# evfro/polara

Measured on AMD Instinct MI355X. Metric: users scored/sec + SVD build time, ML-20M rank-50 PureSVD, higher is better.
Workload: dtype bf16x3; 1 GPU; ML-20M-shaped synthetic 138493 x 26744, ~2e7 nnz, 10 levels (BASELINE.json metric / configs[2]), PureSVD rank=50, top-10, all users scored; n_items=26744, nnz=19975287, rank=50, topk=10, prune=True, launch=python, passes on 2 streams

## Files before the change

polara_amd/csrc/score.hip:

```cpp
#include "pk_common.h"
#include "pk_settle.h"
#include <math.h>
#include <stdlib.h>

typedef float f32x16 __attribute__((ext_vector_type(16)));
typedef __bf16 bf16x8 __attribute__((ext_vector_type(8)));

#define RING 16

#define PK_IDX_FLOOR (-2)
#define PK_TILE_NONE 0xffffffff00000000ull

template <int K, int J, int S>
constexpr unsigned long long pk_wave_stage_mask() {
    unsigned long long m = 0;
    for (int l = 0; l < 64; ++l) {
        const int i = l + 64 * S;
        if (((i & J) == 0) == ((i & K) == 0)) m |= 1ull << l;
    }
    return m;
}
template <int SLOTS, int K, int J>
__device__ __forceinline__ void pk_sort32_stage(unsigned (&key)[SLOTS]) {
    if constexpr (J >= 64) {
        const unsigned hi = key[0] > key[1] ? key[0] : key[1], lo = key[0] > key[1] ? key[1] : key[0];
        key[0] = hi;
        key[1] = lo;
    } else {
        unsigned other[SLOTS];
#pragma unroll
        for (int s = 0; s < SLOTS; ++s) other[s] = (unsigned)pk_lane_xor<J>((int)key[s]);
        {
            const unsigned hi = key[0] > other[0] ? key[0] : other[0], lo = key[0] > other[0] ? other[0] : key[0];
            key[0] = __builtin_amdgcn_inverse_ballot_w64(pk_wave_stage_mask<K, J, 0>()) ? hi : lo;
        }
        if constexpr (SLOTS == 2) {
            const unsigned hi = key[1] > other[1] ? key[1] : other[1], lo = key[1] > other[1] ? other[1] : key[1];
            key[1] = __builtin_amdgcn_inverse_ballot_w64(pk_wave_stage_mask<K, J, 1>()) ? hi : lo;
        }
    }
}
template <int SLOTS, int K, int J>
__device__ __forceinline__ void pk_sort32_merge(unsigned (&key)[SLOTS]) {
    pk_sort32_stage<SLOTS, K, J>(key);
    if constexpr (J > 1) pk_sort32_merge<SLOTS, K, (J >> 1)>(key);
}
template <int SLOTS, int K>
__device__ __forceinline__ void pk_sort32_levels(unsigned (&key)[SLOTS]) {
    if constexpr (K > 2) pk_sort32_levels<SLOTS, (K >> 1)>(key);
    pk_sort32_merge<SLOTS, K, (K >> 1)>(key);
}
template <int SLOTS>
__device__ __forceinline__ void pk_sort32_wave_desc(unsigned (&key)[SLOTS]) {
    static_assert(SLOTS == 1 || SLOTS == 2, "pk_sort32_wave_desc: 64 or 128 elements");
    pk_sort32_levels<SLOTS, 64 * SLOTS>(key);
}

template <int K, int J>
constexpr unsigned long long pk_half_stage_mask() {
    unsigned long long m = 0;
    for (int l = 0; l < 64; ++l) {
        const int t = l & 31;
        if (((t & J) == 0) == ((t & K) == 0)) m |= 1ull << l;
    }
    return m;
}
template <int K, int J>
__device__ __forceinline__ void pk_sort32_half_merge(unsigned &key) {
    const unsigned other = (unsigned)pk_lane_xor<J>((int)key);
    const unsigned hi = key > other ? key : other, lo = key > other ? other : key;
    key = __builtin_amdgcn_inverse_ballot_w64(pk_half_stage_mask<K, J>()) ? hi : lo;
    if constexpr (J > 1) pk_sort32_half_merge<K, (J >> 1)>(key);
}
template <int K>
__device__ __forceinline__ void pk_sort32_half_levels(unsigned &key) {
    if constexpr (K > 2) pk_sort32_half_levels<(K >> 1)>(key);
    pk_sort32_half_merge<K, (K >> 1)>(key);
}
__device__ __forceinline__ unsigned pk_float_order(float x) {
    const unsigned u = __float_as_uint(x);
    return (u & 0x80000000u) ? ~u : (u | 0x80000000u);
}

__device__ __forceinline__ unsigned pk_bf16_rne(float x) {
    unsigned u = __float_as_uint(x);
    u += 0x7fffu + ((u >> 16) & 1u);
    return u >> 16;
}
__device__ __forceinline__ void pk_split_bf16(float x, unsigned &hi, unsigned &lo) {
    hi = pk_bf16_rne(x);
    lo = pk_bf16_rne(x - __uint_as_float(hi << 16));
}

struct LaneState {
    int64_t sp;
    float tau;
    int cnt;
};
#define PK_LANE_DONE (-1)

__host__ __device__ constexpr bool pk_top_in_lds(int nstep, int kc) { return kc <= 32 || nstep > 8; }
__host__ __device__ constexpr int pk_ring_rows(int nstep, int kc) { return kc == 16 ? 8 : ((nstep > 8 && kc == 64) ? 2 * RING : RING); }
__host__ __device__ constexpr size_t pk_score_lds_bytes(int nstep, int kc) {
    return (size_t)(4 * pk_ring_rows(nstep, kc) * 64 + (pk_top_in_lds(nstep, kc) ? 4 * 32 * kc : 1)) * sizeof(uint2);
}
struct SeenDense {
    const unsigned *mask;
    const int32_t *skip;
    int tiles;
};

struct UserRows {
    const double *E;
    int64_t ld;
    int K;
    const double *extra;
    int64_t extra_ld;
    double extra_scale;
    float *bound_out;
};

struct SettleExit {
    int topk;
    double vmax;
    const float *item_norm;
    int64_t *out_idx;
    const int64_t *out_perm;
    int32_t *flags;
    int32_t *open_list;
    int32_t *open_count;
};

struct ExitCtx {
    SettleExit sx;
    const int64_t *seen_ptr;
    const double *extra;
    int64_t extra_ld;
    int64_t n_users;
    int K;
};
#define PK_EXIT_CTX_BYTES 128
static_assert(sizeof(ExitCtx) <= PK_EXIT_CTX_BYTES, "ExitCtx: one 128-byte LDS slot per wave");
__host__ __device__ constexpr size_t pk_score_settle_lds_bytes(int nstep, int kc) { return pk_score_lds_bytes(nstep, kc) + 4 * PK_EXIT_CTX_BYTES; }

template <int NSTEP, int KC, bool STRIDED, bool DENSE, bool SETTLE = false>
__global__ __launch_bounds__(256) void score_candidates_kernel(
    const float4 *__restrict__ Vp, const float4 *__restrict__ Ep, int64_t n_users, int n_items,
    int n_tiles, int split_tiles, int chunk_begin, int chunk_tiles,
    const int64_t *__restrict__ seen_ptr, const unsigned long long *__restrict__ seen_tiles,
    const int32_t *__restrict__ seen_ntiles,
    float *__restrict__ cand_score, int32_t *__restrict__ cand_idx,
    LaneState *__restrict__ st_lane, uint2 *__restrict__ st_ring,
    const float *__restrict__ user_bound, const float *__restrict__ tile_bound, SeenDense dense,
    int tile_base, int slot_base, const LaneState *__restrict__ floor_state, int boot_tiles, UserRows rows, SettleExit sx) {
    constexpr int KQ = 2 * NSTEP;
    constexpr bool PAIRED = (KC == 16);
    constexpr int RG = pk_ring_rows(NSTEP, KC);
    constexpr int SLOTS = (2 * RG + KC + 63) / 64;
    constexpr bool TOP_LDS = pk_top_in_lds(NSTEP, KC);
    extern __shared__ __attribute__((aligned(16))) uint2 pk_score_lds[];
    constexpr int NW = 4;

    const int lane = threadIdx.x & 63;
    const int wave = __builtin_amdgcn_readfirstlane((int)(threadIdx.x >> 6));
    const int64_t group_raw = (int64_t)blockIdx.x * NW + wave;
    if (group_raw * 32 >= n_users) return;
    const int64_t group = group_raw;
    uint2(*ring)[64] = reinterpret_cast<uint2(*)[64]>(pk_score_lds + wave * (RG * 64));
    uint2 *top = pk_score_lds + NW * RG * 64 + (TOP_LDS ? wave * (32 * KC) : 0);
    constexpr int CTX_AT = NW * RG * 64 + NW * 32 * KC;
    if constexpr (SETTLE) {
        if (lane == 0) {
            ExitCtx *cx = reinterpret_cast<ExitCtx *>(pk_score_lds + CTX_AT + wave * (PK_EXIT_CTX_BYTES / 8));
            cx->sx = sx;
            cx->seen_ptr = seen_ptr;
            cx->extra = rows.extra;
            cx->extra_ld = rows.extra_ld;
            cx->n_users = n_users;
            cx->K = rows.K;
        }
    }

    const int split = STRIDED ? (int)blockIdx.y : 0;
    const int S = STRIDED ? (int)gridDim.y : 1;
    const int64_t n_groups = (n_users + 31) / 32;
    const int t_lo = tile_base + split;
    const int tile_begin = t_lo + chunk_begin * S;
    const int tile_stop = (chunk_begin + chunk_tiles < split_tiles) ? t_lo + (chunk_begin + chunk_tiles) * S : n_tiles;
    const int tile_end = (tile_stop < n_tiles) ? tile_stop : n_tiles;
    const bool first = (chunk_begin == 0);
    const bool last = (tile_stop >= n_tiles);
    if (!first && tile_begin >= n_tiles) return;

    const int ul = lane & 31, hi = lane >> 5;
    const int64_t user = group * 32 + ul;
    const int64_t slot = (int64_t)(slot_base + split) * n_groups + group;
    float *my_score = cand_score + slot * 32 * KC;
    int32_t *my_idx = cand_idx + slot * 32 * KC;

    float4 e[KQ];
    float en_rows = -1.0f;
    if (rows.E) {
        double *buf = reinterpret_cast<double *>(&ring[0][0]);
        double ss = 0.0;
#pragma unroll
        for (int s = 0; s < NSTEP; ++s) {
            __builtin_amdgcn_wave_barrier();
#pragma unroll
            for (int p = 0; p < 4; ++p) {
                const int rr = 8 * p + (lane >> 3);
                const int kk = 16 * s + 2 * (lane & 7);
                const int64_t grow = group * 32 + rr;
                double2 v = make_double2(0.0, 0.0);
                if (grow < n_users && kk < rows.K) {
                    const double *g = rows.E + grow * rows.ld + kk;
                    if (kk + 1 < rows.K) v = *reinterpret_cast<const double2 *>(g);
                    else v.x = g[0];
                }
                *reinterpret_cast<double2 *>(buf + rr * 16 + 2 * (lane & 7)) = v;
            }
            __builtin_amdgcn_wave_barrier();
            unsigned bh[8], bl[8];
            const double *mine = buf + ul * 16 + 8 * hi;
#pragma unroll
            for (int j = 0; j < 8; ++j) {
                const double x = mine[j];
                ss = fma(x, x, ss);
                pk_split_bf16((float)x, bh[j], bl[j]);
            }
            e[2 * s] = __builtin_bit_cast(float4, make_uint4(bh[0] | (bh[1] << 16), bh[2] | (bh[3] << 16), bh[4] | (bh[5] << 16), bh[6] | (bh[7] << 16)));
            e[2 * s + 1] = __builtin_bit_cast(float4, make_uint4(bl[0] | (bl[1] << 16), bl[2] | (bl[3] << 16), bl[4] | (bl[5] << 16), bl[6] | (bl[7] << 16)));
        }
        __builtin_amdgcn_wave_barrier();
        ss += pk_lane_xor<32>(ss);
        if (user < n_users) {
            double b = sqrt(ss) * (1.0 + 1e-6);
            if (rows.extra) b += rows.extra_scale * rows.extra[user * rows.extra_ld];
            en_rows = (float)(b * (1.0 + 1e-7));
            if (rows.bound_out && chunk_begin == 0 && hi == 0 && (!STRIDED || blockIdx.y == 0)) rows.bound_out[user] = en_rows;
        }
    } else {
#pragma unroll
        for (int q = 0; q < KQ; ++q) e[q] = Ep[(group * KQ + q) * 64 + lane];
    }

    int64_t sp = 0, se = 0;
    unsigned long long nxt = PK_TILE_NONE, nxt2 = PK_TILE_NONE, nxt3 = PK_TILE_NONE;
    float tau = -INFINITY;
    int cnt = 0;
    const bool prune = (user_bound != nullptr || rows.E != nullptr) && tile_bound != nullptr;
    const float en = (prune && user < n_users) ? (rows.E ? en_rows : user_bound[user]) : -1.0f;
    bool pruned = false;
    int exit_tile = tile_end;
    const bool has_seen = (seen_ptr != nullptr && user < n_users);
    if (has_seen) {
        sp = seen_ptr[user];
        se = sp + seen_ntiles[user];
    }
    LaneState *my_state = st_lane + slot * 64 + lane;
    uint2 *my_ring_state = st_ring + slot * (RING * 64);
    float tau_floor = -INFINITY;
    if constexpr (STRIDED) {
        if (floor_state) {
            const LaneState fs = floor_state[group * 64 + lane];
            if ((int)fs.sp < tile_base) {
                if (first) {
                    for (int s = lane; s < 32 * KC; s += 64) {
                        my_score[s] = -INFINITY;
                        my_idx[s] = -1;
                    }
                    LaneState ls;
                    ls.sp = fs.sp;
                    ls.tau = fs.tau;
                    ls.cnt = PK_LANE_DONE;
                    *my_state = ls;
                }
                return;
            }
            tau_floor = fs.tau;
            tau = tau_floor;
        }
    }
    const int dense_tiles = (DENSE && seen_ptr != nullptr) ? dense.tiles : 0;
    const unsigned *dense_row = dense_tiles ? dense.mask + ((int64_t)group * dense_tiles) * 32 + ul : nullptr;
    if (DENSE && first && has_seen && dense_tiles) sp += dense.skip[user];
    if (first) {
        if (has_seen && t_lo > 0 && !(DENSE && dense_tiles >= t_lo)) {
            int64_t lo = sp, hi_ = se;
            while (lo < hi_) {
                const int64_t mid = (lo + hi_) >> 1;
                if ((unsigned)(seen_tiles[mid] >> 32) < (unsigned)t_lo) lo = mid + 1; else hi_ = mid;
            }
            sp = lo;
        }
        for (int s = lane; s < 32 * KC; s += 64) {
            if (TOP_LDS) {
                top[s] = make_uint2(__float_as_uint(-INFINITY), 0xffffffffu);
            } else {
                my_score[s] = -INFINITY;
                my_idx[s] = -1;
            }
        }
    } else {
        const LaneState ls = *my_state;
        if (ls.cnt == PK_LANE_DONE) {
            return;
        }
        if (TOP_LDS)
            for (int s = lane; s < 32 * KC; s += 64) top[s] = make_uint2(__float_as_uint(my_score[s]), (unsigned)my_idx[s]);
        if (has_seen) sp = ls.sp;
        tau = ls.tau;
        tau_floor = fmaxf(tau_floor, tau);
        cnt = ls.cnt;
        const int cmax = __builtin_amdgcn_readfirstlane((int)__reduce_max_sync(~0ull, cnt));
        for (int i = 0; i < cmax; ++i) ring[i][lane] = my_ring_state[i * 64 + lane];
    }
    if (has_seen) {
        if (sp < se) nxt = seen_tiles[sp];
        if (sp + 1 < se) nxt2 = seen_tiles[sp + 1];
        if (sp + 2 < se) nxt3 = seen_tiles[sp + 2];
    }

    auto flush_user = [&](int x) {
        if (TOP_LDS) {
            __builtin_amdgcn_wave_barrier();
        } else {
            __builtin_amdgcn_fence(__ATOMIC_RELEASE, "workgroup");
            __builtin_amdgcn_wave_barrier();
        }
        const int c_lo = __builtin_amdgcn_readlane(cnt, x);
        const int c_hi = __builtin_amdgcn_readlane(cnt, x + 32);
        if (!TOP_LDS) __builtin_amdgcn_fence(__ATOMIC_ACQUIRE, "workgroup");
        if constexpr (SLOTS == 2 && KC == 64) {
            constexpr unsigned SRC_MASK = 127u;
            float ka = -INFINITY, kb = -INFINITY;
            int va = PK_IDX_NONE, vb = PK_IDX_NONE;
            if (TOP_LDS) {
                const uint2 r = top[x * KC + lane];
                if ((int)r.y >= 0) {
                    ka = __uint_as_float(r.x);
                    va = (int)r.y;
                }
            } else {
                const int iv = my_idx[x * KC + lane];
                if (iv >= 0) {
                    ka = my_score[x * KC + lane];
                    va = iv;
                }
            }
            if (lane < RG) {
                if (lane < c_lo) {
                    const uint2 r = ring[lane][x];
                    kb = __uint_as_float(r.x);
                    vb = (int)r.y;
                }
            } else if (lane < 2 * RG) {
                if (lane - RG < c_hi) {
                    const uint2 r = ring[lane - RG][x + 32];
                    kb = __uint_as_float(r.x);
                    vb = (int)r.y;
                }
            }
            unsigned qa = (pk_float_order(ka) & ~SRC_MASK) | (unsigned)(127 - lane);
            unsigned qb[1] = {(pk_float_order(kb) & ~SRC_MASK) | (unsigned)lane};
            pk_sort32_wave_desc<1>(qb);
            const unsigned qr = (unsigned)__shfl((int)qb[0], 63 - lane, 64);
            unsigned q[1] = {qa > qr ? qa : qr};
            pk_sort32_merge<1, 64, 32>(q);
            const int code = (int)(q[0] & SRC_MASK);
            const int src = (code >= 64) ? 127 - code : code;
            const float fa = __shfl(ka, src, 64), fb = __shfl(kb, src, 64);
            const int ia = __shfl(va, src, 64), ib = __shfl(vb, src, 64);
            const float fk = (code >= 64) ? fa : fb;
            const int fv = (code >= 64) ? ia : ib;
            const int iv = (fv == PK_IDX_NONE) ? -1 : fv;
            if (TOP_LDS) {
                top[x * KC + lane] = make_uint2(__float_as_uint(fk), (unsigned)iv);
            } else {
                my_score[x * KC + lane] = fk;
                my_idx[x * KC + lane] = iv;
            }
            const float ntau = __int_as_float(__builtin_amdgcn_readlane(__float_as_int(fk), KC - 1));
            if (ul == x) {
                tau = fmaxf(ntau, tau_floor);
                cnt = 0;
            }
            __builtin_amdgcn_wave_barrier();
            return;
        }
        float key[SLOTS];
        int val[SLOTS];
#pragma unroll
        for (int s = 0; s < SLOTS; ++s) {
            const int i = lane + 64 * s;
            float k = -INFINITY;
            int v = PK_IDX_NONE;
            if (i < RG) {
                if (i < c_lo) {
                    uint2 r = ring[i][x];
                    k = __uint_as_float(r.x);
                    v = (int)r.y;
                }
            } else if (i < 2 * RG) {
                if (i - RG < c_hi) {
                    uint2 r = ring[i - RG][x + 32];
                    k = __uint_as_float(r.x);
                    v = (int)r.y;
                }
            } else if (i < 2 * RG + KC) {
                const int t = i - 2 * RG;
                if (TOP_LDS) {
                    const uint2 r = top[x * KC + t];
                    if ((int)r.y >= 0) {
                        k = __uint_as_float(r.x);
                        v = (int)r.y;
                    }
                } else {
                    const int iv = my_idx[x * KC + t];
                    if (iv >= 0) {
                        k = my_score[x * KC + t];
                        v = iv;
                    }
                }
            }
            key[s] = k;
            val[s] = v;
        }
        constexpr unsigned SRC_MASK = 64u * SLOTS - 1u;
        unsigned k32[SLOTS];
#pragma unroll
        for (int s = 0; s < SLOTS; ++s) k32[s] = (pk_float_order(key[s]) & ~SRC_MASK) | (unsigned)(lane + 64 * s);
        pk_sort32_wave_desc<SLOTS>(k32);
        {
            float ok[SLOTS];
            int ov[SLOTS];
#pragma unroll
            for (int s = 0; s < SLOTS; ++s) {
                const int src = (int)(k32[s] & SRC_MASK);
                float fk = __shfl(key[0], src & 63, 64);
                int fv = __shfl(val[0], src & 63, 64);
                if constexpr (SLOTS == 2) {
                    const float fk1 = __shfl(key[1], src & 63, 64);
                    const int fv1 = __shfl(val[1], src & 63, 64);
                    if (src >= 64) {
                        fk = fk1;
                        fv = fv1;
                    }
                }
                ok[s] = fk;
                ov[s] = fv;
            }
#pragma unroll
            for (int s = 0; s < SLOTS; ++s) {
                key[s] = ok[s];
                val[s] = ov[s];
            }
        }
#pragma unroll
        for (int s = 0; s < SLOTS; ++s) {
            const int i = lane + 64 * s;
            if (i < KC) {
                const int iv = (val[s] == PK_IDX_NONE) ? -1 : val[s];
                if (TOP_LDS) {
                    top[x * KC + i] = make_uint2(__float_as_uint(key[s]), (unsigned)iv);
                } else {
                    my_score[x * KC + i] = key[s];
                    my_idx[x * KC + i] = iv;
                }
            }
        }
        const float ntau = __int_as_float(
            __builtin_amdgcn_readlane(__float_as_int(key[(KC - 1) / 64]), (KC - 1) & 63));
        if (ul == x) {
            tau = fmaxf(ntau, tau_floor);
            cnt = 0;
        }
        __builtin_amdgcn_wave_barrier();
    };
    auto flush_pair = [&](int x, int y) {
        __builtin_amdgcn_wave_barrier();
        const int t = lane & 31;
        const int yy = (y >= 0) ? y : x;
        const int cx_lo = __builtin_amdgcn_readlane(cnt, x), cx_hi = __builtin_amdgcn_readlane(cnt, x + 32);
        const int cy_lo = __builtin_amdgcn_readlane(cnt, yy), cy_hi = __builtin_amdgcn_readlane(cnt, yy + 32);
        const int u = hi ? yy : x;
        const int c_lo = hi ? cy_lo : cx_lo, c_hi = hi ? cy_hi : cx_hi;
        const bool act = !hi || y >= 0;
        float k = -INFINITY;
        int v = PK_IDX_NONE;
        if (act) {
            if (t < KC) {
                const uint2 r = top[u * KC + t];
                if ((int)r.y >= 0) {
                    k = __uint_as_float(r.x);
                    v = (int)r.y;
                }
            } else if (t < KC + RG) {
                if (t - KC < c_lo) {
                    const uint2 r = ring[t - KC][u];
                    k = __uint_as_float(r.x);
                    v = (int)r.y;
                }
            } else if (t - KC - RG < c_hi) {
                const uint2 r = ring[t - KC - RG][u + 32];
                k = __uint_as_float(r.x);
                v = (int)r.y;
            }
        }
        unsigned key = (pk_float_order(k) & ~31u) | (unsigned)t;
        pk_sort32_half_levels<32>(key);
        const int src = (lane & 32) | (int)(key & 31u);
        k = __shfl(k, src, 64);
        v = __shfl(v, src, 64);
        if (act && t < KC) top[u * KC + t] = make_uint2(__float_as_uint(k), (unsigned)((v == PK_IDX_NONE) ? -1 : v));
        const float tx = __int_as_float(__builtin_amdgcn_readlane(__float_as_int(k), KC - 1));
        const float ty = __int_as_float(__builtin_amdgcn_readlane(__float_as_int(k), 32 + KC - 1));
        if (ul == x) {
            tau = fmaxf(tx, tau_floor);
            cnt = 0;
        }
        if (y >= 0 && ul == y) {
            tau = fmaxf(ty, tau_floor);
            cnt = 0;
        }
        __builtin_amdgcn_wave_barrier();
    };
    auto flush_set = [&](unsigned um) {
        if constexpr (PAIRED) {
            while (um) {
                const int x = __builtin_ctz(um);
                um &= um - 1;
                int y = -1;
                if (um) {
                    y = __builtin_ctz(um);
                    um &= um - 1;
                }
                flush_pair(x, y);
            }
        } else {
            while (um) {
                const int x = __builtin_ctz(um);
                um &= um - 1;
                flush_user(x);
            }
        }
    };

    auto load_frags = [&](int tile, float4(&dst)[KQ]) {
        const float4 *vp = Vp + ((int64_t)tile * KQ) * 64 + lane;
#pragma unroll
        for (int q = 0; q < KQ; ++q) dst[q] = vp[q * 64];
    };
    unsigned m_dense = 0;
    unsigned long long pend = PK_TILE_NONE;
    bool has_pend = false;
    auto take_pending = [&]() {
        if (has_pend) nxt3 = (sp + 2 < se) ? pend : PK_TILE_NONE;
        has_pend = false;
    };
    auto walk_mask = [&](int tile) -> unsigned {
        const int j0 = tile * 32, jend = j0 + 32;
        unsigned mask = 0;
        if constexpr (DENSE) {
            if (tile < dense_tiles) {
                mask = m_dense;
                if (jend > n_items) mask |= ~0u << (n_items - j0);
                return mask;
            }
        }
        if (S > 1) {
            while (__any((unsigned)(nxt >> 32) < (unsigned)tile)) {
                take_pending();
                if ((unsigned)(nxt >> 32) < (unsigned)tile) {
                    ++sp;
                    nxt = nxt2;
                    nxt2 = nxt3;
                    nxt3 = (sp + 2 < se) ? seen_tiles[sp + 2] : PK_TILE_NONE;
                }
            }
        }
        const bool hit = (unsigned)(nxt >> 32) == (unsigned)tile;
        if (__any(hit)) {
            take_pending();
            if (hit) {
                mask = (unsigned)nxt;
                ++sp;
                nxt = nxt2;
                nxt2 = nxt3;
                nxt3 = PK_TILE_NONE;
            }
            pend = seen_tiles[(hit && sp + 2 < se) ? sp + 2 : 0];
            has_pend = hit;
        }
        if (jend > n_items) mask |= ~0u << (n_items - j0);
        return mask;
    };
    auto push_candidates = [&](const float(&acc)[16], int j0) {
#pragma unroll
        for (int r = 0; r < 16; ++r) {
            bool c = acc[r] > tau;
            if (__any(c)) {
                if (__any(c && cnt == RG)) {
                    const unsigned long long full = __ballot(cnt == RG);
                    unsigned um = (unsigned)(full | (full >> 32));
                    if (PAIRED && (__builtin_popcount(um) & 1)) {
                        const unsigned long long part = __ballot(2 * cnt >= RG);
                        const unsigned cand = (unsigned)(part | (part >> 32)) & ~um;
                        if (cand) um |= 1u << __builtin_ctz(cand);
                    }
                    flush_set(um);
                    c = acc[r] > tau;
                }
                if (c) {
                    ring[cnt][lane] = make_uint2(__float_as_uint(acc[r]),
                                                 (unsigned)(j0 + (r & 3) + 8 * (r >> 2) + 4 * hi));
                    ++cnt;
                }
            }
        }
    };
    auto score_tile_roll = [&](float4(&a)[KQ], int next_tile) -> f32x16 {
        f32x16 acc;
#pragma unroll
        for (int r = 0; r < 16; ++r) acc[r] = 0.0f;
        const float4 *vp = Vp + ((int64_t)next_tile * KQ) * 64 + lane;
#pragma unroll
        for (int sidx = 0; sidx < NSTEP; ++sidx) {
            const bf16x8 vh = __builtin_bit_cast(bf16x8, a[2 * sidx]), vl = __builtin_bit_cast(bf16x8, a[2 * sidx + 1]);
            const bf16x8 eh = __builtin_bit_cast(bf16x8, e[2 * sidx]), el = __builtin_bit_cast(bf16x8, e[2 * sidx + 1]);
            acc = __builtin_amdgcn_mfma_f32_32x32x16_bf16(vh, eh, acc, 0, 0, 0);
            acc = __builtin_amdgcn_mfma_f32_32x32x16_bf16(vh, el, acc, 0, 0, 0);
            acc = __builtin_amdgcn_mfma_f32_32x32x16_bf16(vl, eh, acc, 0, 0, 0);
            a[2 * sidx] = vp[(2 * sidx) * 64];
            a[2 * sidx + 1] = vp[(2 * sidx + 1) * 64];
        }
        return acc;
    };
    if (first && boot_tiles > 0 && floor_state == nullptr) {
        constexpr int BL = KC / 2;
        constexpr int BG = KC / 8;
        float bl[BL];
#pragma unroll
        for (int i = 0; i < BL; ++i) bl[i] = -INFINITY;
        const int64_t sp0 = sp;
        const unsigned long long n0 = nxt, n1 = nxt2, n2 = nxt3;
        float4 a_nxt[KQ];
        load_frags((tile_begin < n_tiles) ? tile_begin : 0, a_nxt);
        unsigned m_nxt = 0u;
        if constexpr (DENSE) m_nxt = (tile_begin < dense_tiles) ? dense_row[(int64_t)tile_begin * 32] : 0u;
        for (int i = 0, tile = tile_begin; i < boot_tiles && tile < tile_end; ++i, tile += S) {
            {
                if constexpr (DENSE) {
                    m_dense = m_nxt;
                    m_nxt = (tile + S < dense_tiles) ? dense_row[(int64_t)(tile + S) * 32] : 0u;
                }
                f32x16 acc;
                acc = score_tile_roll(a_nxt, (tile + S < tile_end) ? tile + S : tile);
                const unsigned m2 = walk_mask(tile) >> (4 * hi);
#pragma unroll
                for (int g = 0; g < BG; ++g) {
                    float x = -INFINITY;
#pragma unroll
                    for (int r = g * (16 / BG); r < (g + 1) * (16 / BG); ++r)
                        x = fmaxf(x, (m2 & (1u << ((r & 3) + 8 * (r >> 2)))) ? -INFINITY : acc[r]);
#pragma unroll
                    for (int i2 = 0; i2 < BL; ++i2) {
                        const float up = fmaxf(bl[i2], x);
                        x = fminf(bl[i2], x);
                        bl[i2] = up;
                    }
                }
            }
        }
        float t0 = bl[KC / 2 - 1];
        t0 = fminf(t0, __int_as_float(pk_lane_xor<32>(__float_as_int(t0))));
        if (t0 > -INFINITY) {
            t0 = fminf(t0 - fabsf(t0) * 2.4e-7f, t0 - 1e-37f);
            tau_floor = fmaxf(tau_floor, t0);
            tau = fmaxf(tau, tau_floor);
        }
        sp = sp0;
        nxt = n0;
        nxt2 = n1;
        nxt3 = n2;
        has_pend = false;
    }
    {
        {
        float4 a_nxt[KQ];
        load_frags((tile_begin < n_tiles) ? tile_begin : 0, a_nxt);
        unsigned m_nxt = 0u;
        if constexpr (DENSE) m_nxt = (tile_begin < dense_tiles) ? dense_row[(int64_t)tile_begin * 32] : 0u;
        float tb = prune ? tile_bound[(tile_begin < n_tiles) ? tile_begin : 0] : 0.0f;
        int step = 0;
        for (int tile = tile_begin; tile < tile_end; tile += S, ++step) {
            if (prune) {
                const bool open = en * tb > tau;
                const unsigned long long ob = __ballot(open);
                if (ob == 0ull) {
                    pruned = true;
                    exit_tile = tile;
                    break;
                } else {
                    if (((STRIDED ? step : tile) & 7) == 7 && __popcll(ob) <= 16) {
                        const unsigned long long pend = __ballot(cnt > 0);
                        flush_set((unsigned)(ob | (ob >> 32)) & (unsigned)(pend | (pend >> 32)));
                    }
                    tb = tile_bound[(tile + S < n_tiles) ? tile + S : tile];
                }
            }
            {
                if constexpr (DENSE) {
                    m_dense = m_nxt;
                    m_nxt = (tile + S < dense_tiles) ? dense_row[(int64_t)(tile + S) * 32] : 0u;
                }
                f32x16 acc;
                acc = score_tile_roll(a_nxt, (tile + S < tile_end) ? tile + S : tile);
                const unsigned mask = walk_mask(tile);
                float m_all = fmaxf(acc[0], acc[1]);
#pragma unroll
                for (int r = 2; r < 16; ++r) m_all = fmaxf(m_all, acc[r]);
                if (__any(m_all > tau)) {
                    float sc[16];
                    float m = m_all;
                    if (__any(mask != 0)) {
                        const unsigned m2 = mask >> (4 * hi);
#pragma unroll
                        for (int r = 0; r < 16; ++r)
                            sc[r] = (m2 & (1u << ((r & 3) + 8 * (r >> 2)))) ? -INFINITY : acc[r];
                        m = fmaxf(sc[0], sc[1]);
#pragma unroll
                        for (int r = 2; r < 16; ++r) m = fmaxf(m, sc[r]);
                    } else {
#pragma unroll
                        for (int r = 0; r < 16; ++r) sc[r] = acc[r];
                    }
                    if (__any(m > tau)) push_candidates(sc, tile * 32);
                }
            }
        }
        }
    }

    if (!last && !pruned) {
        if constexpr (RG > RING) {
            const unsigned long long over = __ballot(cnt > RING);
            flush_set((unsigned)(over | (over >> 32)));
        }
        LaneState ls;
        ls.sp = sp;
        ls.tau = tau;
        ls.cnt = cnt;
        *my_state = ls;
        const int cmax = __builtin_amdgcn_readfirstlane((int)__reduce_max_sync(~0ull, cnt));
        __builtin_amdgcn_wave_barrier();
        for (int i = 0; i < cmax; ++i) my_ring_state[i * 64 + lane] = ring[i][lane];
        if (TOP_LDS)
            for (int s = lane; s < 32 * KC; s += 64) {
                const uint2 r = top[s];
                my_score[s] = __uint_as_float(r.x);
                my_idx[s] = (int)r.y;
            }
        return;
    }
    {
        const unsigned long long some = __ballot(cnt > 0);
        flush_set((unsigned)(some | (some >> 32)));
    }
    const unsigned long long floored = (floor_state == nullptr) ? __ballot(tau_floor > -INFINITY) : 0ull;
    unsigned settled_users = 0u;
    if constexpr (SETTLE) {
        static_assert(TOP_LDS && !STRIDED && (KC == 16 || KC == 32), "settle at exit: single sweep, lists in LDS, KC <= 32");
        constexpr int UPP = 64 / KC;
        const int sl = (int)__builtin_amdgcn_mbcnt_hi(~0u, __builtin_amdgcn_mbcnt_lo(~0u, 0u));
        int cx_at = CTX_AT + __builtin_amdgcn_readfirstlane((int)(threadIdx.x >> 6)) * (PK_EXIT_CTX_BYTES / 8);
        asm volatile("" : "+s"(cx_at));
        __builtin_amdgcn_wave_barrier();
        const ExitCtx cx = *reinterpret_cast<const ExitCtx *>(pk_score_lds + cx_at);
        const SettleExit &sx = cx.sx;
        const int64_t n_users = cx.n_users;
        const int64_t sgroup = (int64_t)blockIdx.x * NW + __builtin_amdgcn_readfirstlane((int)(threadIdx.x >> 6));
        const int su = sl & 31;
        const int64_t suser = sgroup * 32 + su;
        const int t = sl % KC, seg = sl / KC;
        double c_own = 0.0;
        int can_own = 0;
        int64_t irow_own = 0;
        if (suser < n_users) {
            c_own = pk_settle_coeff(cx.K, en, cx.extra[suser * cx.extra_ld]);
            const int64_t n_seen = cx.seen_ptr ? cx.seen_ptr[suser + 1] - cx.seen_ptr[suser] : 0;
            can_own = (n_items - n_seen >= sx.topk) ? 1 : 0;
            irow_own = sx.out_perm ? sx.out_perm[suser] : suser;
        }
        static_assert((size_t)RG * 64 * sizeof(uint2) >= (size_t)32 * KC * sizeof(float), "norms fit the ring area");
        float *nrm = reinterpret_cast<float *>(&ring[0][0]);
        __builtin_amdgcn_wave_barrier();
#pragma unroll
        for (int i = 0; i < KC / 2; ++i) {
            const int iv = (int)top[sl + 64 * i].y;
            nrm[sl + 64 * i] = (sx.item_norm && iv >= 0) ? sx.item_norm[iv] : 0.0f;
        }
        __builtin_amdgcn_wave_barrier();
#pragma unroll 1
        for (int p = 0; p < 32 / UPP; ++p) {
            const int x = p * UPP + seg;
            const uint2 r = top[x * KC + t];
            const uint2 rl = top[x * KC + KC - 1];
            float n_me = nrm[x * KC + t];
            double ts = -INFINITY;
            int ti = PK_IDX_NONE;
            if ((int)r.y >= 0) {
                ts = (double)__uint_as_float(r.x);
                ti = (int)r.y;
            }
            const double tau32 = ((int)rl.y >= 0) ? (double)__uint_as_float(rl.x) : -INFINITY;
            const bool unbounded = (int)rl.y < 0 && ((floored >> x) & 1ull);
            pk_bitonic_seg<KC, 1>(ts, ti, t, n_me);
            const double c = __shfl(c_own, x, 64);
            const int can = __shfl(can_own, x, 64);
            const long long irow = __shfl((long long)irow_own, x, 64);
            const double d_max = c * sx.vmax;
            double d_me = d_max;
            if (sx.item_norm && ti != PK_IDX_NONE) d_me = pk_settle_item_err(c, sx.vmax, n_me);
            const int k_lane = seg * KC + sx.topk - 1;
            const double s_nb = __shfl(ts, (sl + 1) & 63, 64), d_nb = __shfl(d_me, (sl + 1) & 63, 64);
            const double s_next = (t + 1 < KC) ? s_nb : -INFINITY;
            const double d_next = (t + 1 < KC) ? d_nb : d_max;
            const double s_kk = __shfl(ts, k_lane, 64), d_kk = __shfl(d_me, k_lane, 64);
            bool open = (t < sx.topk) ? !(ts - s_next > d_me + d_next) : !(s_kk - ts > d_kk + d_me);
            if (tau32 > -INFINITY) open = open || !(s_kk - pk_settle_tau_cert(tau32) > d_kk + d_max);
            open = open || unbounded || !can;
            const unsigned long long ob = __ballot(open);
            constexpr unsigned long long SEG_ONES = (1ull << KC) - 1ull;
            if (((ob >> (seg * KC)) & SEG_ONES) == 0ull) {
                if (t < sx.topk) sx.out_idx[irow * sx.topk + t] = (ti == PK_IDX_NONE) ? -1 : (int64_t)ti;
                if (t == 0) sx.flags[sgroup * 32 + x] = PK_FLAG_SETTLED;
            }
#pragma unroll
            for (int g = 0; g < UPP; ++g)
                if (((ob >> (g * KC)) & SEG_ONES) == 0ull) settled_users |= 1u << (p * UPP + g);
        }
        const unsigned open_users = (unsigned)__ballot(suser < n_users) & ~settled_users;
        if (open_users) {
            int base = 0;
            if (sl == 0) base = atomicAdd(sx.open_count, __builtin_popcount(open_users));
            base = __builtin_amdgcn_readfirstlane(base);
            const int64_t at = (int64_t)base + __builtin_popcount(open_users & ((1u << su) - 1u));
            if (sl < 32 && ((open_users >> su) & 1u) && at >= 0 && at < n_users) sx.open_list[at] = (int32_t)suser;
        }
    }
    if (TOP_LDS) {
        __builtin_amdgcn_wave_barrier();
        for (int s = lane; s < 32 * KC; s += 64) {
            if (SETTLE && ((settled_users >> (s / KC)) & 1u)) continue;
            const uint2 r = top[s];
            int iv = (int)r.y;
            if ((s % KC) == KC - 1 && iv < 0 && ((floored >> (s / KC)) & 1ull)) iv = PK_IDX_FLOOR;
            my_score[s] = __uint_as_float(r.x);
            my_idx[s] = iv;
        }
    } else if (floored) {
        __builtin_amdgcn_fence(__ATOMIC_RELEASE, "workgroup");
        __builtin_amdgcn_wave_barrier();
        __builtin_amdgcn_fence(__ATOMIC_ACQUIRE, "workgroup");
        if (hi == 0 && tau_floor > -INFINITY && my_idx[ul * KC + KC - 1] < 0) my_idx[ul * KC + KC - 1] = PK_IDX_FLOOR;
    }
    {
        LaneState ls;
        ls.sp = exit_tile;
        ls.tau = tau;
        ls.cnt = PK_LANE_DONE;
        *my_state = ls;
    }
}

static const int kNstepSet[] = {1, 2, 3, 4, 5, 6, 7, 8, 10, 13, 16};

static int pk_nstep(int K) {
    const int need = (K + 15) / 16;
    for (int n : kNstepSet)
        if (n >= need) return n;
    return 0;
}

extern "C" int32_t pk_pack_kq(int32_t K) {
    const int n = pk_nstep(K);
    return n ? 2 * n : 0;
}

extern "C" int64_t pk_pack_elems(int64_t n, int32_t K) {
    const int kq = pk_pack_kq(K);
    return pk_ceil_div(n, 32) * kq * 64 * 4;
}

__device__ __forceinline__ void pk_pack_step(const double *__restrict__ r, bool live, int K, int s, int h, uint4 &ghi, uint4 &glo,
                                             double *sumsq) {
    unsigned hi[8], lo[8];
#pragma unroll
    for (int j = 0; j < 8; ++j) {
        const int k = 16 * s + 8 * h + j;
        const double x = (live && k < K) ? r[k] : 0.0;
        if (sumsq) *sumsq = fma(x, x, *sumsq);
        pk_split_bf16((float)x, hi[j], lo[j]);
    }
    ghi = make_uint4(hi[0] | (hi[1] << 16), hi[2] | (hi[3] << 16), hi[4] | (hi[5] << 16), hi[6] | (hi[7] << 16));
    glo = make_uint4(lo[0] | (lo[1] << 16), lo[2] | (lo[3] << 16), lo[4] | (lo[5] << 16), lo[6] | (lo[7] << 16));
}

__global__ __launch_bounds__(256) void pack_frag_kernel(int64_t n, int K, int kq, const double *__restrict__ src,
                                                        int64_t ld, uint4 *__restrict__ dst, int64_t total) {
    const int64_t t = (int64_t)blockIdx.x * blockDim.x + threadIdx.x;
    if (t >= total) return;
    const int ns = kq / 2;
    const int lane = (int)(t & 63);
    const int64_t ts = t >> 6;
    const int s = (int)(ts % ns);
    const int64_t tile = ts / ns;
    const int64_t row = tile * 32 + (lane & 31);
    uint4 ghi, glo;
    pk_pack_step(src + (row < n ? row : 0) * ld, row < n, K, s, lane >> 5, ghi, glo, nullptr);
    dst[(tile * kq + 2 * s) * 64 + lane] = ghi;
    dst[(tile * kq + 2 * s + 1) * 64 + lane] = glo;
}

__global__ __launch_bounds__(256) void pack_frag_bound_kernel(int64_t n, int K, int kq, const double *__restrict__ src,
                                                              int64_t ld, uint4 *__restrict__ dst,
                                                              float *__restrict__ bound,
                                                              const double *__restrict__ extra, int64_t extra_ld,
                                                              double extra_scale, int64_t n_tiles) {
    __shared__ __attribute__((aligned(16))) double s_tile[4][32 * 16];
    const int lane = threadIdx.x & 63;
    const int wave = threadIdx.x >> 6;
    const int64_t tile = (int64_t)blockIdx.x * 4 + wave;
    if (tile >= n_tiles) return;
    const int64_t row = tile * 32 + (lane & 31);
    const int h = lane >> 5;
    const bool live = row < n;
    const double *r = src + (live ? row : 0) * ld;
    double ss = 0.0;
    const bool staged = ((ld & 1) == 0) && ((((uintptr_t)src) & 15) == 0);
    for (int s = 0; s < kq / 2; ++s) {
        uint4 ghi, glo;
        if (staged) {
            double *buf = s_tile[wave];
            __builtin_amdgcn_wave_barrier();
#pragma unroll
            for (int p = 0; p < 4; ++p) {
                const int rr = 8 * p + (lane >> 3);
                const int kk = 16 * s + 2 * (lane & 7);
                const int64_t grow = tile * 32 + rr;
                double2 v = make_double2(0.0, 0.0);
                if (grow < n && kk < K) {
                    const double *g = src + grow * ld + kk;
                    if (kk + 1 < K) v = *reinterpret_cast<const double2 *>(g);
                    else v.x = g[0];
                }
                *reinterpret_cast<double2 *>(buf + rr * 16 + 2 * (lane & 7)) = v;
            }
            __builtin_amdgcn_wave_barrier();
            unsigned hi[8], lo[8];
            const double *mine = buf + (lane & 31) * 16 + 8 * h;
#pragma unroll
            for (int j = 0; j < 8; ++j) {
                const double x = mine[j];
                ss = fma(x, x, ss);
                pk_split_bf16((float)x, hi[j], lo[j]);
            }
            ghi = make_uint4(hi[0] | (hi[1] << 16), hi[2] | (hi[3] << 16), hi[4] | (hi[5] << 16), hi[6] | (hi[7] << 16));
            glo = make_uint4(lo[0] | (lo[1] << 16), lo[2] | (lo[3] << 16), lo[4] | (lo[5] << 16), lo[6] | (lo[7] << 16));
        } else {
            pk_pack_step(r, live, K, s, h, ghi, glo, &ss);
        }
        dst[(tile * kq + 2 * s) * 64 + lane] = ghi;
        dst[(tile * kq + 2 * s + 1) * 64 + lane] = glo;
    }
    ss += pk_lane_xor<32>(ss);
    if (live && h == 0) {
        double b = sqrt(ss) * (1.0 + 1e-6);
        if (extra) b += extra_scale * extra[row * extra_ld];
        bound[row] = (float)(b * (1.0 + 1e-7));
    }
}

extern "C" int pk_pack_frag_bound_f32(void *stream, int64_t n, int32_t K, const double *src_dev, int64_t ld,
                                      float *dst_dev, float *bound_dev, const double *extra_dev, int64_t extra_ld,
                                      double extra_scale) {
    const int kq = pk_pack_kq(K);
    PK_REQUIRE(n >= 1 && K >= 1 && kq > 0, "pk_pack_frag_bound_f32: n=%lld K=%d unsupported (K <= 256)", (long long)n, K);
    PK_REQUIRE(ld >= K && ((uintptr_t)dst_dev % 16) == 0 && bound_dev, "pk_pack_frag_bound_f32: bad ld / alignment / pointers");
    const int64_t n_tiles = pk_ceil_div(n, 32);
    hipLaunchKernelGGL(pack_frag_bound_kernel, dim3((unsigned)pk_ceil_div(n_tiles, 4)), dim3(256), 0, pk_stream(stream), n,
                       K, kq, src_dev, ld, reinterpret_cast<uint4 *>(dst_dev), bound_dev, extra_dev, extra_ld,
                       extra_scale, n_tiles);
    PK_CHECK_LAUNCH("pack_frag_bound_kernel");
    return PK_OK;
}

extern "C" int pk_pack_frag_f32(void *stream, int64_t n, int32_t K, const double *src_dev, int64_t ld,
                                float *dst_dev) {
    const int kq = pk_pack_kq(K);
    PK_REQUIRE(n >= 1 && K >= 1 && kq > 0, "pk_pack_frag_f32: n=%lld K=%d unsupported (K <= 256)", (long long)n, K);
    PK_REQUIRE(ld >= K && ((uintptr_t)dst_dev % 16) == 0, "pk_pack_frag_f32: bad ld / alignment");
    const int64_t total = pk_ceil_div(n, 32) * (kq / 2) * 64;
    hipLaunchKernelGGL(pack_frag_kernel, dim3((unsigned)pk_ceil_div(total, 256)), dim3(256), 0, pk_stream(stream), n,
                       K, kq, src_dev, ld, reinterpret_cast<uint4 *>(dst_dev), total);
    PK_CHECK_LAUNCH("pack_frag_kernel");
    return PK_OK;
}

#define PK_SEEN_CAP 4096
template <bool SORTED>
__global__ __launch_bounds__(256) void seen_tiles_kernel(int64_t n_users, const int64_t *__restrict__ seen_ptr,
                                                         const int32_t *__restrict__ seen_idx,
                                                         unsigned long long *__restrict__ tiles,
                                                         int32_t *__restrict__ ntiles) {
    __shared__ int sort_buf[SORTED ? 1 : 4][SORTED ? 1 : PK_SEEN_CAP];
    const int lane = threadIdx.x & 63;
    const int64_t user = (int64_t)blockIdx.x * 4 + (threadIdx.x >> 6);
    if (user >= n_users) return;
    const int64_t p0 = seen_ptr[user], p1 = seen_ptr[user + 1];
    int *buf = sort_buf[SORTED ? 0 : (threadIdx.x >> 6)];
    if constexpr (!SORTED) {
        const int n = (int)(p1 - p0);
        int N = 64;
        while (N < n) N <<= 1;
        for (int i = lane; i < N; i += 64) buf[i] = (i < n) ? seen_idx[p0 + i] : 0x7fffffff;
        __builtin_amdgcn_wave_barrier();
        for (int k = 2; k <= N; k <<= 1) {
            for (int j = k >> 1; j > 0; j >>= 1) {
                for (int t = lane; t < (N >> 1); t += 64) {
                    const int pos = ((t & ~(j - 1)) << 1) | (t & (j - 1));
                    const int x = buf[pos], y = buf[pos + j];
                    const bool up = (pos & k) == 0;
                    if ((x > y) == up) {
                        buf[pos] = y;
                        buf[pos + j] = x;
                    }
                }
                __builtin_amdgcn_wave_barrier();
            }
        }
    }
    int count = 0;
    bool carry = false;
    unsigned c_tile = 0, c_mask = 0;
    for (int64_t base = p0; base < p1; base += 64) {
// ... 566 lines not shown
```

Baseline: 203.9 million users/s.

## Software-pipeline tile MFMAs with previous tile's mask/top-k work in dense settle sweeps

For selected dense, non-strided settle kernel variants, the boot and main sweep loops are restructured to double-buffer accumulators: the MFMAs for the next tile are issued while the previous tile's masking, max and candidate filtering run, with sched_group_barrier hints interleaving MFMA and VALU work. The aim is to hide MFMA latency behind the selection arithmetic instead of serialising them. It also sets amdgpu_waves_per_eu for these variants to change register and occupancy targets. In exchange, register pressure rises from the two live accumulators, and the code only supports single-stride sweeps.

```diff
diff --git a/polara_amd/csrc/score.hip b/polara_amd/csrc/score.hip
--- a/polara_amd/csrc/score.hip
+++ b/polara_amd/csrc/score.hip
@@ -143,8 +143,37 @@
 static_assert(sizeof(ExitCtx) <= PK_EXIT_CTX_BYTES, "ExitCtx: one 128-byte LDS slot per wave");
 __host__ __device__ constexpr size_t pk_score_settle_lds_bytes(int nstep, int kc) { return pk_score_lds_bytes(nstep, kc) + 4 * PK_EXIT_CTX_BYTES; }
 
+template <int NSTEP, int FROM, int TO>
+__device__ __forceinline__ void pk_tile_mfmas(f32x16 &acc, float4 (&a)[2 * NSTEP], const float4 (&e)[2 * NSTEP], const float4 *vp) {
+    constexpr int M = 3 * NSTEP;
+#pragma unroll
+    for (int j = (FROM < M ? FROM : M); j < (TO < M ? TO : M); ++j) {
+        const int sidx = j / 3, part = j % 3;
+        const bf16x8 vh = __builtin_bit_cast(bf16x8, a[2 * sidx]), vl = __builtin_bit_cast(bf16x8, a[2 * sidx + 1]);
+        const bf16x8 eh = __builtin_bit_cast(bf16x8, e[2 * sidx]), el = __builtin_bit_cast(bf16x8, e[2 * sidx + 1]);
+        if (j == 0) {
+#pragma unroll
+            for (int r = 0; r < 16; ++r) acc[r] = 0.0f;
+        }
+        acc = __builtin_amdgcn_mfma_f32_32x32x16_bf16(part == 2 ? vl : vh, part == 1 ? el : eh, acc, 0, 0, 0);
+        if (part == 2) {
+            a[2 * sidx] = vp[(2 * sidx) * 64];
+            a[2 * sidx + 1] = vp[(2 * sidx + 1) * 64];
+        }
+    }
+}
+__host__ __device__ constexpr bool pk_sweep_overlap(int nstep, int kc, bool strided, bool dense, bool settle) {
+#ifdef PK_SWEEP_PLAIN
+    return false;
+#else
+    return !strided && dense && settle && ((nstep == 4 && kc == 16) || (nstep == 7 && kc == 32));
+#endif
+}
+__host__ __device__ constexpr int pk_sweep_overlap_waves(int nstep) { return nstep <= 4 ? 3 : 2; }
+
 template <int NSTEP, int KC, bool STRIDED, bool DENSE, bool SETTLE = false>
-__global__ __launch_bounds__(256) void score_candidates_kernel(
+__global__ __launch_bounds__(256) __attribute__((amdgpu_waves_per_eu(pk_sweep_overlap(NSTEP, KC, STRIDED, DENSE, SETTLE) ? pk_sweep_overlap_waves(NSTEP) : 1)))
+void score_candidates_kernel(
     const float4 *__restrict__ Vp, const float4 *__restrict__ Ep, int64_t n_users, int n_items,
     int n_tiles, int split_tiles, int chunk_begin, int chunk_tiles,
     const int64_t *__restrict__ seen_ptr, const unsigned long long *__restrict__ seen_tiles,
@@ -154,6 +183,10 @@
     const float *__restrict__ user_bound, const float *__restrict__ tile_bound, SeenDense dense,
     int tile_base, int slot_base, const LaneState *__restrict__ floor_state, int boot_tiles, UserRows rows, SettleExit sx) {
     constexpr int KQ = 2 * NSTEP;
+    constexpr bool OVERLAP = pk_sweep_overlap(NSTEP, KC, STRIDED, DENSE, SETTLE);
+    constexpr int MF = 3 * NSTEP;
+    constexpr int MF_HEAD = MF < 5 ? MF : 5;
+    constexpr int PK_GAP_FILL = 5;
     constexpr bool PAIRED = (KC == 16);
     constexpr int RG = pk_ring_rows(NSTEP, KC);
     constexpr int SLOTS = (2 * RG + KC + 63) / 64;
@@ -648,6 +681,51 @@
         load_frags((tile_begin < n_tiles) ? tile_begin : 0, a_nxt);
         unsigned m_nxt = 0u;
         if constexpr (DENSE) m_nxt = (tile_begin < dense_tiles) ? dense_row[(int64_t)tile_begin * 32] : 0u;
+        if constexpr (OVERLAP) {
+            static_assert(!STRIDED, "overlapped loops: only single sweeps are switched and tested; the S-generic arithmetic (tile + 2 S, step) has not run with S > 1");
+            auto boot_tile = [&](const f32x16 &acc, f32x16 &nacc, int tile) {
+                if constexpr (DENSE) {
+                    m_dense = m_nxt;
+                    m_nxt = (tile + S < dense_tiles) ? dense_row[(int64_t)(tile + S) * 32] : 0u;
+                }
+                const float4 *vp = Vp + ((int64_t)((tile + 2 * S < tile_end) ? tile + 2 * S : tile) * KQ) * 64 + lane;
+                pk_tile_mfmas<NSTEP, 0, 1>(nacc, a_nxt, e, vp);
+                const unsigned m2 = walk_mask(tile) >> (4 * hi);
+                pk_tile_mfmas<NSTEP, 1, MF>(nacc, a_nxt, e, vp);
+#pragma unroll
+                for (int g = 0; g < BG; ++g) {
+                    float x = -INFINITY;
+#pragma unroll
+                    for (int r = g * (16 / BG); r < (g + 1) * (16 / BG); ++r)
+                        x = fmaxf(x, (m2 & (1u << ((r & 3) + 8 * (r >> 2)))) ? -INFINITY : acc[r]);
+#pragma unroll
+                    for (int i2 = 0; i2 < BL; ++i2) {
+                        const float up = fmaxf(bl[i2], x);
+                        x = fminf(bl[i2], x);
+                        bl[i2] = up;
+                    }
+                }
+#pragma unroll
+                for (int j = 1; j < MF; ++j) {
+                    __builtin_amdgcn_sched_group_barrier(0x8, 1, 0);
+                    __builtin_amdgcn_sched_group_barrier(0x2, PK_GAP_FILL, 0);
+                }
+            };
+            f32x16 acc_a, acc_b;
+            const int tile_boot = (tile_begin + (int64_t)boot_tiles * S < tile_end) ? tile_begin + boot_tiles * S : tile_end;
+            if (tile_begin < tile_boot) {
+                const float4 *vp = Vp + ((int64_t)((tile_begin + S < tile_end) ? tile_begin + S : tile_begin) * KQ) * 64 + lane;
+                pk_tile_mfmas<NSTEP, 0, MF>(acc_a, a_nxt, e, vp);
+            }
+            asm volatile("" : "+v"(m_nxt));
+            for (int tile = tile_begin; tile < tile_boot;) {
+                boot_tile(acc_a, acc_b, tile);
+                tile += S;
+                if (tile >= tile_boot) break;
+                boot_tile(acc_b, acc_a, tile);
+                tile += S;
+            }
+        } else
         for (int i = 0, tile = tile_begin; i < boot_tiles && tile < tile_end; ++i, tile += S) {
             {
                 if constexpr (DENSE) {
@@ -693,22 +771,78 @@
         if constexpr (DENSE) m_nxt = (tile_begin < dense_tiles) ? dense_row[(int64_t)tile_begin * 32] : 0u;
         float tb = prune ? tile_bound[(tile_begin < n_tiles) ? tile_begin : 0] : 0.0f;
         int step = 0;
+#define PK_LEAVE_OR_STAY(tile)                                                                              \
+        if (prune) {                                                                                        \
+            const bool open = en * tb > tau;                                                                \
+            const unsigned long long ob = __ballot(open);                                                   \
+            if (ob == 0ull) {                                                                               \
+                pruned = true;                                                                              \
+                exit_tile = tile;                                                                           \
+                break;                                                                                      \
+            } else {                                                                                        \
+                if (((STRIDED ? step : tile) & 7) == 7 && __popcll(ob) <= 16) {                             \
+                    const unsigned long long pend = __ballot(cnt > 0);                                      \
+                    flush_set((unsigned)(ob | (ob >> 32)) & (unsigned)(pend | (pend >> 32)));               \
+                }                                                                                           \
+                tb = tile_bound[(tile + S < n_tiles) ? tile + S : tile];                                    \
+            }                                                                                               \
+        }
+        if constexpr (OVERLAP) {
+            auto tile_front = [&](const f32x16 &acc, f32x16 &nacc, int tile, float(&sc)[16]) -> bool {
+                if constexpr (DENSE) {
+                    m_dense = m_nxt;
+                    m_nxt = (tile + S < dense_tiles) ? dense_row[(int64_t)(tile + S) * 32] : 0u;
+                }
+                const float4 *vp = Vp + ((int64_t)((tile + 2 * S < tile_end) ? tile + 2 * S : tile) * KQ) * 64 + lane;
+                pk_tile_mfmas<NSTEP, 0, 1>(nacc, a_nxt, e, vp);
+                const unsigned mask = walk_mask(tile);
+                pk_tile_mfmas<NSTEP, 1, MF_HEAD>(nacc, a_nxt, e, vp);
+                float m_all = fmaxf(acc[0], acc[1]);
+#pragma unroll
+                for (int r = 2; r < 16; ++r) m_all = fmaxf(m_all, acc[r]);
+#pragma unroll
+                for (int j = 1; j < MF_HEAD; ++j) {
+                    __builtin_amdgcn_sched_group_barrier(0x8, 1, 0);
+                    __builtin_amdgcn_sched_group_barrier(0x2, PK_GAP_FILL, 0);
+                }
+                pk_tile_mfmas<NSTEP, MF_HEAD, MF>(nacc, a_nxt, e, vp);
+                if (__any(m_all > tau)) {
+                    float m = m_all;
+                    if (__any(mask != 0)) {
+                        const unsigned m2 = mask >> (4 * hi);
+#pragma unroll
+                        for (int r = 0; r < 16; ++r)
+                            sc[r] = (m2 & (1u << ((r & 3) + 8 * (r >> 2)))) ? -INFINITY : acc[r];
+                        m = fmaxf(sc[0], sc[1]);
+#pragma unroll
+                        for (int r = 2; r < 16; ++r) m = fmaxf(m, sc[r]);
+                    } else {
+#pragma unroll
+                        for (int r = 0; r < 16; ++r) sc[r] = acc[r];
+                    }
+                    return __any(m > tau);
+                }
+                return false;
+            };
+            f32x16 acc_a, acc_b;
+            if (tile_begin < tile_end) {
+                const float4 *vp = Vp + ((int64_t)((tile_begin + S < tile_end) ? tile_begin + S : tile_begin) * KQ) * 64 + lane;
+                pk_tile_mfmas<NSTEP, 0, MF>(acc_a, a_nxt, e, vp);
+            }
+            asm volatile("" : "+v"(m_nxt));
+            for (int tile = tile_begin; tile < tile_end;) {
+                float sc[16];
+                PK_LEAVE_OR_STAY(tile)
+                if (tile_front(acc_a, acc_b, tile, sc)) push_candidates(sc, tile * 32);
+                tile += S, ++step;
+                if (tile >= tile_end) break;
+                PK_LEAVE_OR_STAY(tile)
+                if (tile_front(acc_b, acc_a, tile, sc)) push_candidates(sc, tile * 32);
+                tile += S, ++step;
+            }
+        } else
         for (int tile = tile_begin; tile < tile_end; tile += S, ++step) {
-            if (prune) {
-                const bool open = en * tb > tau;
-                const unsigned long long ob = __ballot(open);
-                if (ob == 0ull) {
-                    pruned = true;
-                    exit_tile = tile;
-                    break;
-                } else {
-                    if (((STRIDED ? step : tile) & 7) == 7 && __popcll(ob) <= 16) {
-                        const unsigned long long pend = __ballot(cnt > 0);
-                        flush_set((unsigned)(ob | (ob >> 32)) & (unsigned)(pend | (pend >> 32)));
-                    }
-                    tb = tile_bound[(tile + S < n_tiles) ? tile + S : tile];
-                }
-            }
+            PK_LEAVE_OR_STAY(tile)
             {
                 if constexpr (DENSE) {
                     m_dense = m_nxt;
@@ -742,6 +876,7 @@
         }
     }
 
+#undef PK_LEAVE_OR_STAY
     if (!last && !pruned) {
         if constexpr (RG > RING) {
             const unsigned long long over = __ballot(cnt > RING);
```

Result: faster. 209.3 million users/s (median of 4 runs) (+2.6%).
